# wg-perception/tod

Hardware: AMD Instinct MI355X
Metric: frames/sec @ 640x480, 1M-descriptor DB; achieved HBM GB/s on BF-matcher (higher is better)
Workload: dtype fp4 (+-1) x fp4 -> f32 on the matrix cores (exact integers), f32 in the verifier

## Files before the change

### tod_amd/csrc/match_mfma.h

```cpp
#ifdef TOD_K4X_COUNT_WALKS
__device__ unsigned long long g_k4x_blocks[2];
#endif
template <int K, bool MASK, bool IMAX>
__device__ __forceinline__ void mfma_block_test(const mfma_f32x16& acc, float& thr, uint32_t r_lane, uint32_t n_lim,
                                                uint32_t (&best)[K]) {
#ifdef TOD_K4X_COUNT_WALKS
  if (!MASK && (threadIdx.x & 63u) == 0u) atomicAdd(&g_k4x_blocks[0], 1ull);
#endif
  if (!MASK) {
    if (__builtin_amdgcn_ballot_w64(block_reaches<IMAX, false>(acc, thr)) == 0ull) return;
#ifdef TOD_K4X_COUNT_WALKS
    if ((threadIdx.x & 63u) == 0u) atomicAdd(&g_k4x_blocks[1], 1ull);
#endif
  }
#pragma unroll
  for (int i = 0; i < 16; ++i) {
    const uint32_t ri = block_row(i);
    const bool hit = MASK ? (acc[i] > thr && (r_lane | ri) < n_lim) : (acc[i] > thr);
    if (__builtin_amdgcn_ballot_w64(hit) != 0ull) {
      const uint32_t key = (uint32_t)((256.f - acc[i]) * 2097152.f) | r_lane | ri;
      topk_insert<K>(best, hit ? key : 0xFFFFFFFFu);
    }
  }
  thr = fmaxf(thr, thr_of_limit(best[K - 1] >> kLocalBits));
}

template <int K, int SPLIT>
__device__ __forceinline__ bool mfma_block_test_part(mfma_f32x16& acc, const Fp4Row& rows, const Fp4Row& q, float& thr, float& thrp,
                                                     uint32_t r_lane, uint32_t n_lim, uint32_t (&best)[K]) {
  if (__builtin_amdgcn_ballot_w64(block_reaches<true, false>(acc, thrp)) == 0ull) return false;
#pragma unroll
  for (int s = SPLIT; s < 4; ++s) acc = __builtin_amdgcn_mfma_scale_f32_32x32x64_f8f6f4(rows.s[s], q.s[s], acc, 4, 4, 0, 0, 0, 0);
  mfma_block_test<K, false, true>(acc, thr, r_lane, n_lim, best);
  thrp = thr - 64.f * (float)(4 - SPLIT);
  return true;
}

template <int K, int QT, bool MASK, bool IMAX, int SPLIT = 0>
__device__ __forceinline__ uint32_t mfma_step(const Fp4Row& a, Fp4Row& a_next, const uint4& p_next, const Fp4Row (&qb)[QT],
                                              float (&thr)[QT], float (&thrp)[QT], uint32_t (&best)[QT][K], mfma_f32x16& acc_even,
                                              mfma_f32x16& acc_odd, uint32_t r_lane, uint32_t n_lim, const Fp4Consts& kc) {
  constexpr bool HALF = SPLIT != 0;
  uint32_t n_pass = 0;
  static_assert(!(HALF && MASK) && !(HALF && !IMAX) && !(HALF && QT < 4), "split blocks: unmasked steps, integer maximum, >= 4 query blocks");
  static_assert(SPLIT == 0 || SPLIT == 2 || SPLIT == 3, "2 or 3 of the 4 MFMAs first");
#pragma unroll
  for (int t = 0; t < QT; ++t) {
    if (HALF) { if (t & 1) acc_odd = dot_part0<HALF ? SPLIT : 2>(a, qb[t]); else acc_even = dot_part0<HALF ? SPLIT : 2>(a, qb[t]); }
    else { if (t & 1) acc_odd = dot_block(a, qb[t]); else acc_even = dot_block(a, qb[t]); }
#if defined(TOD_K4X_ABLATE) && TOD_K4X_ABLATE == 3
    if (t == 0) { a_next = a; asm volatile("" :: "v"(p_next.x), "v"(p_next.y), "v"(p_next.z), "v"(p_next.w)); }
#else
    if (QT >= 4) {
      if (t == 0) a_next.s[0] = expand_word(p_next.x, kc);
      if (t == 1) a_next.s[1] = expand_word(p_next.y, kc);
      if (t == 2) a_next.s[2] = expand_word(p_next.z, kc);
      if (t == 3) a_next.s[3] = expand_word(p_next.w, kc);
    } else {
      if (t == 0) { a_next.s[0] = expand_word(p_next.x, kc); a_next.s[1] = expand_word(p_next.y, kc); }
      if (t == 1) { a_next.s[2] = expand_word(p_next.z, kc); a_next.s[3] = expand_word(p_next.w, kc); }
    }
#endif
#if defined(TOD_K4X_ABLATE) && TOD_K4X_ABLATE == 2
    if (t == 0) asm volatile("" :: "v"(acc_odd)); else if (t & 1) asm volatile("" :: "v"(acc_even)); else asm volatile("" :: "v"(acc_odd));
#else
    if (HALF) {
      if (t == 0) n_pass += mfma_block_test_part<K, HALF ? SPLIT : 2>(acc_odd, a_next, qb[QT - 1], thr[QT - 1], thrp[QT - 1], r_lane - 32u, n_lim, best[QT - 1]) ? 1u : 0u;
      else n_pass += mfma_block_test_part<K, HALF ? SPLIT : 2>((t & 1) ? acc_even : acc_odd, a, qb[t - 1], thr[t - 1], thrp[t - 1], r_lane, n_lim, best[t - 1]) ? 1u : 0u;
    } else {
      if (t == 0) mfma_block_test<K, MASK, IMAX>(acc_odd, thr[QT - 1], r_lane - 32u, n_lim, best[QT - 1]);
      else mfma_block_test<K, MASK, IMAX>((t & 1) ? acc_even : acc_odd, thr[t - 1], r_lane, n_lim, best[t - 1]);
    }
#endif
  }
  return n_pass;
}

template <int K, int QT, int MODE, bool PF2>
__global__ __launch_bounds__(kBlock, 2) void hamming_topk_mfma(const uint32_t* __restrict__ db,
                                                               const uint32_t* __restrict__ q, uint32_t n_rows,
                                                               uint32_t nq, uint32_t nq_pad, uint32_t rows_per_tile,
                                                               uint32_t n_tiles, uint32_t n_qw, uint32_t n_qw64,
                                                               uint32_t blocks_per_xcd, uint32_t tiles_per_xcd, uint32_t cut,
                                                               uint32_t share_period,
                                                               uint32_t* __restrict__ part, uint32_t* bound,
                                                               uint8_t* __restrict__ stored, uint32_t* half_stats) {
  static_assert(QT % 2 == 0 && QT >= 2, "two query blocks share a 64-query flag byte");
  constexpr bool IMAX = MODE >= 1;
  constexpr int HALF = (MODE >= 2 && QT >= 4) ? MODE : 0;
  constexpr float kPartOff = HALF ? 64.f * (float)(4 - HALF) : 0.f;
  const uint32_t xcd = blockIdx.x & 7u, slot = blockIdx.x >> 3;
  uint32_t tile, qw;
  if (tiles_per_xcd) {
    const uint32_t local = __builtin_amdgcn_readfirstlane(slot * kWavesPerBlock + (threadIdx.x >> 6));
    if (local >= tiles_per_xcd * n_qw) return;
    tile = xcd * tiles_per_xcd + local / n_qw; qw = local % n_qw;
  } else {
    const uint32_t vblock = xcd * blocks_per_xcd + slot;
    const uint32_t item = __builtin_amdgcn_readfirstlane(vblock * kWavesPerBlock + (threadIdx.x >> 6));
    tile = item / n_qw; qw = item % n_qw;
  }
  if (tile >= n_tiles) return;
  const uint32_t lane = threadIdx.x & 63u, c = lane & 31u, h = lane >> 5;
  const uint32_t q0 = qw * (32u * QT);

  const Fp4Consts kc = fp4_consts();
  Fp4Row qb[QT];
  uint32_t best[QT][K];
  float thr[QT], thrp[QT];
#pragma unroll
  for (int t = 0; t < QT; ++t) {
    load_query_block(q, q0 + 32u * t + c, nq, h, qb[t], kc);
#pragma unroll
    for (int j = 0; j < K; ++j) best[t][j] = 0xFFFFFFFFu;
    thr[t] = thr_of_limit(cut);
    thrp[t] = thr[t] - kPartOff;
  }

  const uint32_t row0 = tile * rows_per_tile;
  const uint32_t row_end = min(n_rows, row0 + rows_per_tile);
  const uint32_t n_local = row_end - row0;
  const uint32_t n_full = n_local / 32u, n_steps = (n_local + 31u) / 32u;
  const StepLoader rows(db, row0, n_steps, c, h);
#if defined(TOD_K4X_ABLATE) && TOD_K4X_ABLATE == 1
  auto load_step = [&](uint32_t step) -> uint4 {
    const uint32_t r = rows.first_row(step) + c;
    return uint4{r * 2654435761u, r ^ step, r + h, r * 40503u};
  };
#else
  const StepLoader& load_step = rows;
#endif
  Fp4Row a0, a1;
  {
    const uint4 p = load_step(0);
    expand_row(p, a0, kc);
  }
  uint4 pa = load_step(1), pb = PF2 ? load_step(2) : pa;
  mfma_f32x16 acc_even, acc_odd;
#pragma unroll
  for (int i = 0; i < 16; ++i) acc_odd[i] = kNoBlock;
  uint32_t seen[QT];
#pragma unroll
  for (int t = 0; t < QT; ++t) seen[t] = 0xFFFFFFFFu;
  uint32_t next_share = 2u;

  uint32_t step = 0;
  uint32_t n_pass = 0;
  for (; step + 2u <= n_full; step += 2u) {
    n_pass += mfma_step<K, QT, false, IMAX, HALF>(a0, a1, pa, qb, thr, thrp, best, acc_even, acc_odd, lane_row_base(step, h), n_local, kc);
    if (PF2) {
      pa = load_step(step + 3u);
      n_pass += mfma_step<K, QT, false, IMAX, HALF>(a1, a0, pb, qb, thr, thrp, best, acc_even, acc_odd, lane_row_base(step, h) + 32u, n_local, kc);
      pb = load_step(step + 4u);
    } else {
      pa = load_step(step + 2u);
      n_pass += mfma_step<K, QT, false, IMAX, HALF>(a1, a0, pa, qb, thr, thrp, best, acc_even, acc_odd, lane_row_base(step, h) + 32u, n_local, kc);
      pa = load_step(step + 3u);
    }
    if (step + 2u >= next_share) {
      next_share += share_period;
#pragma unroll
      for (int t = 0; t < QT; ++t) {
        const uint32_t qi = q0 + 32u * t + c;
        uint32_t* my_bound = bound + (qi < nq ? qi : nq - 1u);
        const uint32_t worst_d = best[t][K - 1] >> kLocalBits;
        if (worst_d < (0xFFFFFFFFu >> kLocalBits) && worst_d < seen[t]) atomicMin(my_bound, worst_d);
        if (seen[t] != 0xFFFFFFFFu) { thr[t] = fmaxf(thr[t], thr_of_limit(seen[t] + 1u)); thrp[t] = thr[t] - kPartOff; }
        seen[t] = __hip_atomic_load(my_bound, __ATOMIC_RELAXED, __HIP_MEMORY_SCOPE_AGENT);
      }
    }
  }
  if (HALF && step > 0u) {
    n_pass += mfma_block_test_part<K, HALF ? HALF : 2>(acc_odd, a1, qb[QT - 1], thr[QT - 1], thrp[QT - 1], lane_row_base(step - 1u, h), n_local, best[QT - 1]) ? 1u : 0u;
#pragma unroll
    for (int i = 0; i < 16; ++i) acc_odd[i] = kNoBlock;
    if (lane == 0 && half_stats) { atomicAdd(half_stats, n_pass); atomicAdd(half_stats + 1, step * (uint32_t)QT); }
  }
  for (; step < n_steps; ++step) {
    mfma_step<K, QT, true, IMAX>(a0, a1, pa, qb, thr, thrp, best, acc_even, acc_odd, lane_row_base(step, h), n_local, kc);
    a0 = a1;
    pa = PF2 ? pb : load_step(step + 2u);
  }
  mfma_block_test<K, true, IMAX>(acc_odd, thr[QT - 1], lane_row_base(n_steps - 1u, h), n_local, best[QT - 1]);

#pragma unroll
  for (int t = 0; t < QT; ++t) {
    uint32_t other[K];
#pragma unroll
    for (int j = 0; j < K; ++j) other[j] = __shfl_xor(best[t][j], 32);
#pragma unroll
    for (int j = 0; j < K; ++j) topk_insert<K>(best[t], other[j]);
  }
#pragma unroll
  for (int u = 0; u < QT / 2; ++u) {
    const uint32_t qa = q0 + 64u * u + c, qb2 = qa + 32u;
    const bool any_a = qa < nq && best[2 * u][0] != 0xFFFFFFFFu, any_b = qb2 < nq && best[2 * u + 1][0] != 0xFFFFFFFFu;
    if (__builtin_amdgcn_ballot_w64(any_a || any_b) != 0ull) {
      if (h == 0u) {
#pragma unroll
        for (int j = 0; j < K; ++j) {
          if (qa < nq) part[((size_t)tile * K + j) * nq_pad + qa] = best[2 * u][j];
          if (qb2 < nq) part[((size_t)tile * K + j) * nq_pad + qb2] = best[2 * u + 1][j];
        }
      }
      if (lane == 0) stored[(size_t)tile * n_qw64 + (q0 >> 6) + u] = 0;
    }
  }
}

template <int K, bool IMAX>
__global__ __launch_bounds__(kBlock) void hamming_topk_mfma_q32(const uint32_t* __restrict__ db, const uint32_t* __restrict__ q,
                                                                uint32_t n_rows, uint32_t nq, uint32_t nq_pad, uint32_t rows_per_tile,
                                                                uint32_t n_tiles, uint32_t n_qw64, uint32_t cut, uint32_t share_period,
                                                                uint32_t* __restrict__ part, uint32_t* bound,
                                                                uint8_t* __restrict__ stored) {
  const uint32_t tile = __builtin_amdgcn_readfirstlane(blockIdx.x * kWavesPerBlock + (threadIdx.x >> 6));
  if (tile >= n_tiles) return;
  const uint32_t lane = threadIdx.x & 63u, c = lane & 31u, h = lane >> 5;
  const Fp4Consts kc = fp4_consts();
  Fp4Row qb;
  load_query_block(q, c, nq, h, qb, kc);
  uint32_t best[K];
#pragma unroll
  for (int j = 0; j < K; ++j) best[j] = 0xFFFFFFFFu;
  float thr = thr_of_limit(cut);
  const uint32_t row0 = tile * rows_per_tile;
  const uint32_t n_local = min(n_rows, row0 + rows_per_tile) - row0;
  const uint32_t n_full = n_local / 32u, n_steps = (n_local + 31u) / 32u;
  const uint32_t last_row = n_rows - 1u;
  auto load_step = [&](uint32_t step) -> uint4 {
    const uint32_t r = min(row0 + 32u * min(step, n_steps - 1u) + c, last_row);
    return *reinterpret_cast<const uint4*>(db + (size_t)r * kWords + 4u * h);
  };
  uint4 p0 = load_step(0), p1 = load_step(1), p2 = load_step(2), p3 = load_step(3);
  mfma_f32x16 acc_a, acc_b;
#pragma unroll
  for (int i = 0; i < 16; ++i) acc_b[i] = kNoBlock;
  uint32_t* my_bound = bound + (c < nq ? c : nq - 1u);
  uint32_t seen = 0xFFFFFFFFu, next_share = 2u, step = 0;
  for (; step + 4u <= n_full; step += 4u) {
    Fp4Row a;
    expand_row(p0, a, kc); p0 = load_step(step + 4u);
    acc_a = dot_block(a, qb);
    mfma_block_test<K, false, IMAX>(acc_b, thr, lane_row_base(step - 1u, h), n_local, best);
    expand_row(p1, a, kc); p1 = load_step(step + 5u);
    acc_b = dot_block(a, qb);
    mfma_block_test<K, false, IMAX>(acc_a, thr, lane_row_base(step, h), n_local, best);
    expand_row(p2, a, kc); p2 = load_step(step + 6u);
    acc_a = dot_block(a, qb);
    mfma_block_test<K, false, IMAX>(acc_b, thr, lane_row_base(step, h) + 32u, n_local, best);
    expand_row(p3, a, kc); p3 = load_step(step + 7u);
    acc_b = dot_block(a, qb);
    mfma_block_test<K, false, IMAX>(acc_a, thr, lane_row_base(step, h) + 64u, n_local, best);
    if (step + 4u >= next_share) {
      next_share += share_period;
      const uint32_t worst_d = best[K - 1] >> kLocalBits;
      if (worst_d < (0xFFFFFFFFu >> kLocalBits) && worst_d < seen) atomicMin(my_bound, worst_d);
      if (seen != 0xFFFFFFFFu) thr = fmaxf(thr, thr_of_limit(seen + 1u));
      seen = __hip_atomic_load(my_bound, __ATOMIC_RELAXED, __HIP_MEMORY_SCOPE_AGENT);
    }
  }
  mfma_block_test<K, true, IMAX>(acc_b, thr, lane_row_base(step - 1u, h), step ? n_local : 0u, best);
  for (; step < n_steps; ++step) {
    Fp4Row a;
    expand_row(p0, a, kc);
    p0 = p1; p1 = p2; p2 = p3; p3 = load_step(step + 4u);
    acc_a = dot_block(a, qb);
    mfma_block_test<K, true, IMAX>(acc_a, thr, lane_row_base(step, h), n_local, best);
  }
  uint32_t other[K];
#pragma unroll
  for (int j = 0; j < K; ++j) other[j] = __shfl_xor(best[j], 32);
#pragma unroll
  for (int j = 0; j < K; ++j) topk_insert<K>(best, other[j]);
  if (__builtin_amdgcn_ballot_w64(c < nq && best[0] != 0xFFFFFFFFu) != 0ull) {
    if (h == 0u && c < nq) {
#pragma unroll
      for (int j = 0; j < K; ++j) part[((size_t)tile * K + j) * nq_pad + c] = best[j];
    }
    if (lane == 0) stored[(size_t)tile * n_qw64] = 0;
  }
}

template <int K, int QT, int HALF>
__device__ __forceinline__ void exchange_bounds(uint32_t* bound, uint32_t q0, uint32_t c, uint32_t nq, const uint32_t (&best)[QT][K],
                                                uint32_t (&seen)[QT], float (&thr)[QT], float (&thrp)[QT]) {
  constexpr float kPartOff = HALF ? 64.f * (float)(4 - HALF) : 0.f;
#pragma unroll
  for (int t = 0; t < QT; ++t) {
    const uint32_t qi = q0 + 32u * t + c;
    uint32_t* my_bound = bound + (qi < nq ? qi : nq - 1u);
    const uint32_t worst_d = best[t][K - 1] >> kLocalBits;
    if (worst_d < (0xFFFFFFFFu >> kLocalBits) && worst_d < seen[t]) atomicMin(my_bound, worst_d);
    if (seen[t] != 0xFFFFFFFFu) { thr[t] = fmaxf(thr[t], thr_of_limit(seen[t] + 1u)); thrp[t] = thr[t] - kPartOff; }
    seen[t] = __hip_atomic_load(my_bound, __ATOMIC_RELAXED, __HIP_MEMORY_SCOPE_AGENT);
  }
}
template <int K, int QT>
__device__ __forceinline__ void store_tile_lists(uint32_t (&best)[QT][K], uint32_t tile, uint32_t q0, uint32_t nq, uint32_t nq_pad,
                                                 uint32_t n_qw64, uint32_t lane, uint32_t c, uint32_t h, uint32_t* __restrict__ part,
                                                 uint8_t* __restrict__ stored) {
#pragma unroll
  for (int t = 0; t < QT; ++t) {
    uint32_t other[K];
#pragma unroll
    for (int j = 0; j < K; ++j) other[j] = __shfl_xor(best[t][j], 32);
#pragma unroll
    for (int j = 0; j < K; ++j) topk_insert<K>(best[t], other[j]);
  }
#pragma unroll
  for (int u = 0; u < QT / 2; ++u) {
    const uint32_t qa = q0 + 64u * u + c, qb2 = qa + 32u;
    const bool any_a = qa < nq && best[2 * u][0] != 0xFFFFFFFFu, any_b = qb2 < nq && best[2 * u + 1][0] != 0xFFFFFFFFu;
    if (__builtin_amdgcn_ballot_w64(any_a || any_b) != 0ull) {
      if (h == 0u) {
#pragma unroll
        for (int j = 0; j < K; ++j) {
          if (qa < nq) part[((size_t)tile * K + j) * nq_pad + qa] = best[2 * u][j];
          if (qb2 < nq) part[((size_t)tile * K + j) * nq_pad + qb2] = best[2 * u + 1][j];
        }
      }
      if (lane == 0) stored[(size_t)tile * n_qw64 + (q0 >> 6) + u] = 0;
    }
  }
}

__global__ __launch_bounds__(kBlock) void expand_rows_fp4_kernel(const uint32_t* __restrict__ db, uint32_t n_steps, uint4* __restrict__ out) {
  const uint32_t s = blockIdx.x, m = threadIdx.x >> 6, l = threadIdx.x & 63u;
  if (s >= n_steps) return;
  const Fp4Consts kc = fp4_consts();
  const mfma_i32x8 e = expand_word(db[(size_t)fp4_rows_src_row(s, l) * kWords + fp4_rows_src_word(m, l)], kc);
  *reinterpret_cast<uint4*>(reinterpret_cast<char*>(out) + fp4_rows_offset(s, m, l)) =
      uint4{(uint32_t)e[0], (uint32_t)e[1], (uint32_t)e[2], (uint32_t)e[3]};
}
static_assert(kBlock == 256, "expand_rows_fp4_kernel: one workgroup = the 4 x 64 fragments of a step");

typedef uint32_t fp4_u32x4 __attribute__((ext_vector_type(4)));
struct Fp4StepLoader {
  __amdgpu_buffer_rsrc_t copy;
  uint32_t step0, n_steps, lane_off;
  __device__ __forceinline__ Fp4StepLoader(const uint4* p, uint32_t copy_bytes, uint32_t s0, uint32_t n, uint32_t lane)
      : copy(__builtin_amdgcn_make_buffer_rsrc(const_cast<uint4*>(p), 0, (int)copy_bytes, 0x00020000)), step0(s0), n_steps(n),
        lane_off((uint32_t)fp4_rows_offset(0, 0, lane)) {}
  template <bool M_SCALAR>
  __device__ __forceinline__ mfma_i32x8 load(uint32_t step, uint32_t m) const {
    const uint32_t step_off = (uint32_t)fp4_rows_offset(step0 + min(step, n_steps - 1u), M_SCALAR ? m : 0u, 0);
    const fp4_u32x4 v = __builtin_amdgcn_raw_buffer_load_b128(copy, (int)(lane_off + (M_SCALAR ? 0u : m * kFp4FragBytes)), (int)step_off, 0);
    return mfma_i32x8{(int)v.x, (int)v.y, (int)v.z, (int)v.w, 0, 0, 0, 0};
  }
};

template <int K, int SPLIT>
__device__ __forceinline__ void fp4rows_block_test_part(mfma_f32x16& acc, const Fp4Row& rows, const Fp4Row& q, float& thr, float& thrp,
                                                        uint32_t r_lane, uint32_t n_lim, uint32_t (&best)[K], uint32_t& n_pass) {
  if (__builtin_expect(__builtin_amdgcn_ballot_w64(block_reaches<true, false>(acc, thrp)) == 0ull, 1)) return;
  ++n_pass;
#pragma unroll
  for (int s = SPLIT; s < 4; ++s) acc = __builtin_amdgcn_mfma_scale_f32_32x32x64_f8f6f4(rows.s[s], q.s[s], acc, 4, 4, 0, 0, 0, 0);
  mfma_block_test<K, false, true>(acc, thr, r_lane, n_lim, best);
  thrp = thr - 64.f * (float)(4 - SPLIT);
}

template <int K, int QT, bool MASK, bool IMAX, int SPLIT = 0>
__device__ __forceinline__ void fp4rows_step(const Fp4Row& a, Fp4Row& a_next, const Fp4StepLoader& rows, uint32_t next_step,
                                             const Fp4Row (&qb)[QT], float (&thr)[QT], float (&thrp)[QT], uint32_t (&best)[QT][K],
                                             mfma_f32x16& acc_even, mfma_f32x16& acc_odd, uint32_t r_lane, uint32_t n_lim, uint32_t& n_pass) {
  constexpr bool HALF = SPLIT != 0;
  constexpr int kEarly = HALF ? SPLIT : 4;
  static_assert(!(HALF && MASK) && !(HALF && !IMAX) && QT >= 4, "split blocks: unmasked steps, integer maximum; >= 4 query blocks");
  static_assert(SPLIT == 0 || SPLIT == 2 || SPLIT == 3, "2 or 3 of the 4 MFMAs first");
#pragma unroll
  for (int t = 0; t < QT; ++t) {
    if (HALF) { if (t & 1) acc_odd = dot_part0<HALF ? SPLIT : 2>(a, qb[t]); else acc_even = dot_part0<HALF ? SPLIT : 2>(a, qb[t]); }
    else { if (t & 1) acc_odd = dot_block(a, qb[t]); else acc_even = dot_block(a, qb[t]); }
    if (t == 0) {
#pragma unroll
      for (int m = 0; m < kEarly; ++m) a_next.s[m] = rows.template load<!HALF>(next_step, m);
    }
    if (t == 1) {
#pragma unroll
      for (int m = kEarly; m < 4; ++m) a_next.s[m] = rows.template load<!HALF>(next_step, m);
    }
    if (HALF) {
      if (t == 0) fp4rows_block_test_part<K, HALF ? SPLIT : 2>(acc_odd, a_next, qb[QT - 1], thr[QT - 1], thrp[QT - 1], r_lane - 32u, n_lim, best[QT - 1], n_pass);
      else fp4rows_block_test_part<K, HALF ? SPLIT : 2>((t & 1) ? acc_even : acc_odd, a, qb[t - 1], thr[t - 1], thrp[t - 1], r_lane, n_lim, best[t - 1], n_pass);
    } else {
      if (t == 0) mfma_block_test<K, MASK, IMAX>(acc_odd, thr[QT - 1], r_lane - 32u, n_lim, best[QT - 1]);
      else mfma_block_test<K, MASK, IMAX>((t & 1) ? acc_even : acc_odd, thr[t - 1], r_lane, n_lim, best[t - 1]);
    }
  }
}

template <int K, int QT, int MODE>
__global__ __launch_bounds__(kBlock, 2) void hamming_topk_fp4rows(const uint4* __restrict__ rows_fp4,
                                                                  const uint32_t* __restrict__ q, uint32_t n_rows,
                                                                  uint32_t nq, uint32_t nq_pad, uint32_t rows_per_tile,
                                                                  uint32_t n_tiles, uint32_t n_qw, uint32_t n_qw64,
                                                                  uint32_t blocks_per_xcd, uint32_t tiles_per_xcd, uint32_t cut,
                                                                  uint32_t share_period,
                                                                  uint32_t* __restrict__ part, uint32_t* bound,
                                                                  uint8_t* __restrict__ stored, uint32_t* half_stats) {
  static_assert(QT == 4 || QT == 6, "four or six query blocks per wave: with eight the fragments of two steps do not fit beside them");
  constexpr bool IMAX = MODE >= 1;
  constexpr int HALF = MODE >= 2 ? MODE : 0;
  constexpr float kPartOff = HALF ? 64.f * (float)(4 - HALF) : 0.f;
  const uint32_t xcd = blockIdx.x & 7u, slot = blockIdx.x >> 3;
  uint32_t tile, qw;
  if (tiles_per_xcd) {
    const uint32_t local = __builtin_amdgcn_readfirstlane(slot * kWavesPerBlock + (threadIdx.x >> 6));
    if (local >= tiles_per_xcd * n_qw) return;
    tile = xcd * tiles_per_xcd + local / n_qw; qw = local % n_qw;
  } else {
    const uint32_t vblock = xcd * blocks_per_xcd + slot;
    const uint32_t item = __builtin_amdgcn_readfirstlane(vblock * kWavesPerBlock + (threadIdx.x >> 6));
    tile = item / n_qw; qw = item % n_qw;
  }
  if (tile >= n_tiles) return;
  const uint32_t lane = threadIdx.x & 63u, c = lane & 31u, h = lane >> 5;
  const uint32_t q0 = qw * (32u * QT);

  const Fp4Consts kc = fp4_consts();
  Fp4Row qb[QT];
  uint32_t best[QT][K];
  float thr[QT], thrp[QT];
#pragma unroll
  for (int t = 0; t < QT; ++t) {
    load_query_block(q, q0 + 32u * t + c, nq, h, qb[t], kc);
#pragma unroll
    for (int j = 0; j < K; ++j) best[t][j] = 0xFFFFFFFFu;
    thr[t] = thr_of_limit(cut);
    thrp[t] = thr[t] - kPartOff;
  }

  const uint32_t row0 = tile * rows_per_tile;
  const uint32_t n_local = min(n_rows, row0 + rows_per_tile) - row0;
  const uint32_t n_full = n_local / 32u, n_steps = (n_local + 31u) / 32u;
  const Fp4StepLoader rows(rows_fp4, (uint32_t)fp4_rows_bytes(n_rows), row0 / 32u, n_steps, lane);
  Fp4Row a0, a1;
#pragma unroll
  for (int m = 0; m < 4; ++m) a0.s[m] = rows.template load<false>(0, m);
  a1 = a0;
  mfma_f32x16 acc_even, acc_odd;
#pragma unroll
  for (int i = 0; i < 16; ++i) acc_odd[i] = kNoBlock;
  uint32_t seen[QT];
#pragma unroll
  for (int t = 0; t < QT; ++t) seen[t] = 0xFFFFFFFFu;
  uint32_t next_share = 2u, step = 0, n_pass = 0;
  if (MODE == 2 && QT == 6 && ((slot >> 5) & 1u)) __builtin_amdgcn_s_setprio(1);
  for (; step + 2u <= n_full; step += 2u) {
    fp4rows_step<K, QT, false, IMAX, HALF>(a0, a1, rows, step + 1u, qb, thr, thrp, best, acc_even, acc_odd, lane_row_base(step, h), n_local, n_pass);
    fp4rows_step<K, QT, false, IMAX, HALF>(a1, a0, rows, step + 2u, qb, thr, thrp, best, acc_even, acc_odd, lane_row_base(step, h) + 32u, n_local, n_pass);
    if (step + 2u >= next_share) {
      next_share += share_period;
      exchange_bounds<K, QT, HALF>(bound, q0, c, nq, best, seen, thr, thrp);
    }
  }
  if (HALF && step > 0u) {
    fp4rows_block_test_part<K, HALF ? HALF : 2>(acc_odd, a1, qb[QT - 1], thr[QT - 1], thrp[QT - 1], lane_row_base(step - 1u, h), n_local, best[QT - 1], n_pass);
#pragma unroll
    for (int i = 0; i < 16; ++i) acc_odd[i] = kNoBlock;
    if (lane == 0 && half_stats) { atomicAdd(half_stats, n_pass); atomicAdd(half_stats + 1, step * (uint32_t)QT); }
  }
  for (; step < n_steps; ++step) {
    fp4rows_step<K, QT, true, IMAX>(a0, a1, rows, step + 1u, qb, thr, thrp, best, acc_even, acc_odd, lane_row_base(step, h), n_local, n_pass);
    a0 = a1;
  }
  mfma_block_test<K, true, IMAX>(acc_odd, thr[QT - 1], lane_row_base(n_steps - 1u, h), n_local, best[QT - 1]);
  store_tile_lists<K, QT>(best, tile, q0, nq, nq_pad, n_qw64, lane, c, h, part, stored);
}
```

Baseline: 20830.

## Keep only split-prefix query fragments resident and reload tails on pass

In MODE 2 (two-of-four split), the kernel now holds only the first SPLIT fragments of each query block and of the DB rows in registers. The remaining fragments are reloaded from memory (row tails from the buffer, query words re-expanded) only when a block passes the partial-bound test. This cuts VGPR pressure so occupancy or unrolling can improve, and drops the unconditional loads of the tail row fragments. In exchange, passing blocks pay extra load latency and re-expansion, and the masked remainder loop gets its own path.

Result: faster. 21330, median of 6 (+2.4%).

```diff
diff --git a/tod_amd/csrc/match_mfma.h b/tod_amd/csrc/match_mfma.h
--- a/tod_amd/csrc/match_mfma.h
+++ b/tod_amd/csrc/match_mfma.h
@@ -361,6 +361,40 @@
   thrp = thr - 64.f * (float)(4 - SPLIT);
 }
 
+template <int N>
+struct Fp4Frags { mfma_i32x8 s[N]; };
+template <int N>
+__device__ __forceinline__ mfma_f32x16 dot_frags(const Fp4Frags<N>& a, const Fp4Frags<N>& b) {
+  mfma_f32x16 acc = {0.f, 0.f, 0.f, 0.f, 0.f, 0.f, 0.f, 0.f, 0.f, 0.f, 0.f, 0.f, 0.f, 0.f, 0.f, 0.f};
+#pragma unroll
+  for (int s = 0; s < N; ++s) acc = __builtin_amdgcn_mfma_scale_f32_32x32x64_f8f6f4(a.s[s], b.s[s], acc, 4, 4, 0, 0, 0, 0);
+  return acc;
+}
+__device__ __forceinline__ uint4 load_query_packed(const uint32_t* __restrict__ q, uint32_t qi, uint32_t nq, uint32_t h) {
+  return *reinterpret_cast<const uint4*>(q + (size_t)(qi < nq ? qi : nq - 1u) * kWords + 4u * h);
+}
+__device__ __forceinline__ uint32_t packed_word(const uint4& p, int m) { return m == 0 ? p.x : m == 1 ? p.y : m == 2 ? p.z : p.w; }
+
+template <int K, int SPLIT>
+__device__ __forceinline__ void fp4rows_block_test_part(mfma_f32x16& acc, const Fp4StepLoader& rows, uint32_t own_step,
+                                                        const uint32_t* __restrict__ q, uint32_t qi, uint32_t nq, uint32_t h,
+                                                        const Fp4Consts& kc, float& thr, float& thrp, uint32_t r_lane, uint32_t n_lim,
+                                                        uint32_t (&best)[K], uint32_t& n_pass) {
+  if (__builtin_expect(__builtin_amdgcn_ballot_w64(block_reaches<true, false>(acc, thrp)) == 0ull, 1)) return;
+  ++n_pass;
+  asm volatile("" : "+v"(qi));
+  mfma_i32x8 tail[4 - SPLIT];
+#pragma unroll
+  for (int s = SPLIT; s < 4; ++s) tail[s - SPLIT] = rows.template load<true>(own_step, s);
+  const uint4 p = load_query_packed(q, qi, nq, h);
+#pragma unroll
+  for (int s = SPLIT; s < 4; ++s)
+    acc = __builtin_amdgcn_mfma_scale_f32_32x32x64_f8f6f4(tail[s - SPLIT], expand_word(packed_word(p, s), kc), acc, 4, 4, 0, 0, 0, 0);
+  mfma_block_test<K, false, true>(acc, thr, r_lane, n_lim, best);
+  asm("" : "+v"(thr));
+  thrp = thr - 64.f * (float)(4 - SPLIT);
+}
+
 template <int K, int QT, bool MASK, bool IMAX, int SPLIT = 0>
 __device__ __forceinline__ void fp4rows_step(const Fp4Row& a, Fp4Row& a_next, const Fp4StepLoader& rows, uint32_t next_step,
                                              const Fp4Row (&qb)[QT], float (&thr)[QT], float (&thrp)[QT], uint32_t (&best)[QT][K],
@@ -388,6 +422,44 @@
       if (t == 0) mfma_block_test<K, MASK, IMAX>(acc_odd, thr[QT - 1], r_lane - 32u, n_lim, best[QT - 1]);
       else mfma_block_test<K, MASK, IMAX>((t & 1) ? acc_even : acc_odd, thr[t - 1], r_lane, n_lim, best[t - 1]);
     }
+  }
+}
+
+template <int K, int QT, int SPLIT>
+__device__ __forceinline__ void fp4rows_split_step(const Fp4Frags<SPLIT>& a, Fp4Frags<SPLIT>& a_next, const Fp4StepLoader& rows, uint32_t step,
+                                                   const Fp4Frags<SPLIT> (&qh)[QT], const uint32_t* __restrict__ q, uint32_t q0c, uint32_t nq,
+                                                   uint32_t h, const Fp4Consts& kc, float (&thr)[QT], float (&thrp)[QT],
+                                                   uint32_t (&best)[QT][K], mfma_f32x16& acc_even, mfma_f32x16& acc_odd, uint32_t r_lane,
+                                                   uint32_t n_lim, uint32_t& n_pass) {
+  static_assert(SPLIT == 2 || SPLIT == 3, "2 or 3 of the 4 MFMAs first");
+  static_assert(QT >= 4 && QT % 2 == 0, "the pending block alternates between two accumulators");
+#pragma unroll
+  for (int t = 0; t < QT; ++t) {
+    if (t & 1) acc_odd = dot_frags(a, qh[t]); else acc_even = dot_frags(a, qh[t]);
+    if (t == 0) {
+#pragma unroll
+      for (int m = 0; m < SPLIT; ++m) a_next.s[m] = rows.template load<false>(step + 1u, m);
+    }
+    if (t == 0) fp4rows_block_test_part<K, SPLIT>(acc_odd, rows, step - 1u, q, q0c + 32u * (QT - 1), nq, h, kc, thr[QT - 1], thrp[QT - 1], r_lane - 32u, n_lim, best[QT - 1], n_pass);
+    else fp4rows_block_test_part<K, SPLIT>((t & 1) ? acc_even : acc_odd, rows, step, q, q0c + 32u * (t - 1), nq, h, kc, thr[t - 1], thrp[t - 1], r_lane, n_lim, best[t - 1], n_pass);
+  }
+}
+
+template <int K, int QT, int SPLIT>
+__device__ __forceinline__ void fp4rows_split_masked_step(const Fp4Row& a, const Fp4Frags<SPLIT> (&qh)[QT], const uint32_t (&qtail)[QT][4 - SPLIT],
+                                                          const Fp4Consts& kc, float (&thr)[QT], uint32_t (&best)[QT][K],
+                                                          mfma_f32x16& acc_even, mfma_f32x16& acc_odd, uint32_t r_lane, uint32_t n_lim) {
+#pragma unroll
+  for (int t = 0; t < QT; ++t) {
+    Fp4Frags<SPLIT> ah;
+#pragma unroll
+    for (int s = 0; s < SPLIT; ++s) ah.s[s] = a.s[s];
+    mfma_f32x16 acc = dot_frags(ah, qh[t]);
+#pragma unroll
+    for (int s = SPLIT; s < 4; ++s) acc = __builtin_amdgcn_mfma_scale_f32_32x32x64_f8f6f4(a.s[s], expand_word(qtail[t][s - SPLIT], kc), acc, 4, 4, 0, 0, 0, 0);
+    if (t & 1) acc_odd = acc; else acc_even = acc;
+    if (t == 0) mfma_block_test<K, true, true>(acc_odd, thr[QT - 1], r_lane - 32u, n_lim, best[QT - 1]);
+    else mfma_block_test<K, true, true>((t & 1) ? acc_even : acc_odd, thr[t - 1], r_lane, n_lim, best[t - 1]);
   }
 }
 
@@ -420,12 +492,21 @@
   const uint32_t q0 = qw * (32u * QT);
 
   const Fp4Consts kc = fp4_consts();
-  Fp4Row qb[QT];
+  constexpr bool TAILS = MODE == 2;
+  constexpr int NF = TAILS ? HALF : 4;
+  using Frags = typename std::conditional<TAILS, Fp4Frags<NF>, Fp4Row>::type;
+  Frags qb[QT];
   uint32_t best[QT][K];
   float thr[QT], thrp[QT];
 #pragma unroll
   for (int t = 0; t < QT; ++t) {
-    load_query_block(q, q0 + 32u * t + c, nq, h, qb[t], kc);
+    if constexpr (TAILS) {
+      const uint4 p = load_query_packed(q, q0 + 32u * t + c, nq, h);
+#pragma unroll
+      for (int m = 0; m < NF; ++m) qb[t].s[m] = expand_word(packed_word(p, m), kc);
+    } else {
+      load_query_block(q, q0 + 32u * t + c, nq, h, qb[t], kc);
+    }
 #pragma unroll
     for (int j = 0; j < K; ++j) best[t][j] = 0xFFFFFFFFu;
     thr[t] = thr_of_limit(cut);
@@ -436,9 +517,9 @@
   const uint32_t n_local = min(n_rows, row0 + rows_per_tile) - row0;
   const uint32_t n_full = n_local / 32u, n_steps = (n_local + 31u) / 32u;
   const Fp4StepLoader rows(rows_fp4, (uint32_t)fp4_rows_bytes(n_rows), row0 / 32u, n_steps, lane);
-  Fp4Row a0, a1;
-#pragma unroll
-  for (int m = 0; m < 4; ++m) a0.s[m] = rows.template load<false>(0, m);
+  Frags a0, a1;
+#pragma unroll
+  for (int m = 0; m < NF; ++m) a0.s[m] = rows.template load<false>(0, m);
   a1 = a0;
   mfma_f32x16 acc_even, acc_odd;
 #pragma unroll
@@ -449,22 +530,56 @@
   uint32_t next_share = 2u, step = 0, n_pass = 0;
   if (MODE == 2 && QT == 6 && ((slot >> 5) & 1u)) __builtin_amdgcn_s_setprio(1);
   for (; step + 2u <= n_full; step += 2u) {
-    fp4rows_step<K, QT, false, IMAX, HALF>(a0, a1, rows, step + 1u, qb, thr, thrp, best, acc_even, acc_odd, lane_row_base(step, h), n_local, n_pass);
-    fp4rows_step<K, QT, false, IMAX, HALF>(a1, a0, rows, step + 2u, qb, thr, thrp, best, acc_even, acc_odd, lane_row_base(step, h) + 32u, n_local, n_pass);
+    if constexpr (TAILS) {
+      fp4rows_split_step<K, QT, NF>(a0, a1, rows, step, qb, q, q0 + c, nq, h, kc, thr, thrp, best, acc_even, acc_odd, lane_row_base(step, h), n_local, n_pass);
+      fp4rows_split_step<K, QT, NF>(a1, a0, rows, step + 1u, qb, q, q0 + c, nq, h, kc, thr, thrp, best, acc_even, acc_odd, lane_row_base(step, h) + 32u, n_local, n_pass);
+    } else {
+      fp4rows_step<K, QT, false, IMAX, HALF>(a0, a1, rows, step + 1u, qb, thr, thrp, best, acc_even, acc_odd, lane_row_base(step, h), n_local, n_pass);
+      fp4rows_step<K, QT, false, IMAX, HALF>(a1, a0, rows, step + 2u, qb, thr, thrp, best, acc_even, acc_odd, lane_row_base(step, h) + 32u, n_local, n_pass);
+    }
     if (step + 2u >= next_share) {
       next_share += share_period;
       exchange_bounds<K, QT, HALF>(bound, q0, c, nq, best, seen, thr, thrp);
     }
   }
-  if (HALF && step > 0u) {
-    fp4rows_block_test_part<K, HALF ? HALF : 2>(acc_odd, a1, qb[QT - 1], thr[QT - 1], thrp[QT - 1], lane_row_base(step - 1u, h), n_local, best[QT - 1], n_pass);
-#pragma unroll
-    for (int i = 0; i < 16; ++i) acc_odd[i] = kNoBlock;
-    if (lane == 0 && half_stats) { atomicAdd(half_stats, n_pass); atomicAdd(half_stats + 1, step * (uint32_t)QT); }
-  }
-  for (; step < n_steps; ++step) {
-    fp4rows_step<K, QT, true, IMAX>(a0, a1, rows, step + 1u, qb, thr, thrp, best, acc_even, acc_odd, lane_row_base(step, h), n_local, n_pass);
-    a0 = a1;
+  if constexpr (TAILS) {
+    if (step > 0u) {
+      fp4rows_block_test_part<K, NF>(acc_odd, rows, step - 1u, q, q0 + c + 32u * (QT - 1), nq, h, kc, thr[QT - 1], thrp[QT - 1], lane_row_base(step - 1u, h), n_local, best[QT - 1], n_pass);
+#pragma unroll
+      for (int i = 0; i < 16; ++i) acc_odd[i] = kNoBlock;
+      if (lane == 0 && half_stats) { atomicAdd(half_stats, n_pass); atomicAdd(half_stats + 1, step * (uint32_t)QT); }
+    }
+    if (step < n_steps) {
+      uint32_t qtail[QT][4 - NF];
+#pragma unroll
+      for (int t = 0; t < QT; ++t) {
+        const uint4 p = load_query_packed(q, q0 + 32u * t + c, nq, h);
+#pragma unroll
+        for (int m = NF; m < 4; ++m) qtail[t][m - NF] = packed_word(p, m);
+      }
+      Fp4Row a, a_next;
+#pragma unroll
+      for (int m = 0; m < NF; ++m) a.s[m] = a0.s[m];
+#pragma unroll
+      for (int m = NF; m < 4; ++m) a.s[m] = rows.template load<false>(step, m);
+      for (; step < n_steps; ++step) {
+#pragma unroll
+        for (int m = 0; m < 4; ++m) a_next.s[m] = rows.template load<false>(step + 1u, m);
+        fp4rows_split_masked_step<K, QT, NF>(a, qb, qtail, kc, thr, best, acc_even, acc_odd, lane_row_base(step, h), n_local);
+        a = a_next;
+      }
+    }
+  } else {
+    if (HALF && step > 0u) {
+      fp4rows_block_test_part<K, HALF ? HALF : 2>(acc_odd, a1, qb[QT - 1], thr[QT - 1], thrp[QT - 1], lane_row_base(step - 1u, h), n_local, best[QT - 1], n_pass);
+#pragma unroll
+      for (int i = 0; i < 16; ++i) acc_odd[i] = kNoBlock;
+      if (lane == 0 && half_stats) { atomicAdd(half_stats, n_pass); atomicAdd(half_stats + 1, step * (uint32_t)QT); }
+    }
+    for (; step < n_steps; ++step) {
+      fp4rows_step<K, QT, true, IMAX>(a0, a1, rows, step + 1u, qb, thr, thrp, best, acc_even, acc_odd, lane_row_base(step, h), n_local, n_pass);
+      a0 = a1;
+    }
   }
   mfma_block_test<K, true, IMAX>(acc_odd, thr[QT - 1], lane_row_base(n_steps - 1u, h), n_local, best[QT - 1]);
   store_tile_lists<K, QT>(best, tile, q0, nq, nq_pad, n_qw64, lane, c, h, part, stored);
```
